# n7koirala/image_matching

Measured on AMD Instinct MI355X. Metric: encrypted DB vectors matched/sec (HyDia indexScenario, CKKS N=2^15), higher is better.
Workload: dtype u64

## Files before the change

### image_matching_amd/csrc/context.cpp

```cpp
#include <algorithm>
#include <cmath>
#include <cstdio>
#include <cstdlib>
#include <cstring>

#include <sys/stat.h>

#include "hydia_core.h"

namespace hydia {

u64 mulmod_u64(u64 a, u64 b, u64 q) { return (u64)(((u128)a * b) % q); }
u64 powmod_u64(u64 a, u64 e, u64 q) {
    u64 r = 1 % q;
    a %= q;
    for (; e; e >>= 1) {
        if (e & 1) r = mulmod_u64(r, a, q);
        a = mulmod_u64(a, a, q);
    }
    return r;
}
u64 invmod_u64(u64 a, u64 q) { return powmod_u64(a % q, q - 2, q); }

static bool miller_rabin(u64 n) {
// ... 336 lines not shown
        tabs.p2_wg_sync = getenv("HYDIA_P2_WG_SYNC") ? 1 : 0;
        tabs.no_tw_lds = getenv("HYDIA_NO_TW_LDS") ? 1 : 0;
    }
    modup_per_digit = getenv("HYDIA_MODUP_PER_DIGIT") != nullptr;
    loop_a_separate_ip = getenv("HYDIA_LOOPA_SEPARATE_IP") != nullptr;
    loop_a_int_ip = getenv("HYDIA_LOOPA_INT_IP") != nullptr;
    loop_a_limb_fastest = getenv("HYDIA_LOOPA_LIMB_FASTEST") != nullptr;
    relin_separate_intt = getenv("HYDIA_RELIN_SEPARATE_INTT") != nullptr;
    tabs.pm_mask = 0;
    if (!getenv("HYDIA_NTT_INT") && !getenv("HYDIA_NTT_NO_PM"))
        for (int m = 0; m < nT; m++)
            if (!((tabs.fp_mask >> m) & 1u) && mod[m].q < (1ull << 60) && (1ull << 60) - mod[m].q < (1ull << 24)) tabs.pm_mask |= 1u << m;
    if (const char *e = getenv("HYDIA_TENSOR_BPP")) tensor_bpp = std::max(1, atoi(e));
    if (const char *e = getenv("HYDIA_TENSOR_NW")) tensor_nw = atoi(e);
    merge_rescale = getenv("HYDIA_NO_MERGE_RESCALE") == nullptr;
    fuse_ip = getenv("HYDIA_NO_FUSE_IP") == nullptr;
    fork_products = getenv("HYDIA_NO_FORK") == nullptr;
    fuse_loop_a = getenv("HYDIA_NO_FUSE_LOOPA") == nullptr;
    colfuse = getenv("HYDIA_NO_COLFUSE") == nullptr;
    if (const char *e = getenv("HYDIA_MATVEC")) {
        if (e[0] == 'h') matvec_mode = 1;
        else if (e[0] == 'b') matvec_mode = bsgs_babies();
        else if (e[0] >= '1' && e[0] <= '9') matvec_mode = babies_for(1, atoi(e));
        else matvec_mode = 0;
    }
    rot_packed = getenv("HYDIA_KEYS_UNPACKED") == nullptr;
    db_packed = getenv("HYDIA_DB_UNPACKED") == nullptr;
    db_seq_ok = getenv("HYDIA_DB_CT_MAJOR") == nullptr;
    for (int j = 1; j < nQ; j++)
        if (q[j] >> 48) db_packed = false;
// ... 594 lines not shown
```

### image_matching_amd/csrc/evaluator.cpp

```cpp
#include <algorithm>
#include <cmath>
#include <cstring>

#include "hydia_core.h"

#include <exception>

namespace hydia {

static u64 shoup_h(u64 w, u64 q) { return (u64)(((u128)w << 64) / q); }

void op_bytes(const char *op, size_t N, double transforms, double other_bytes) {
    hk::ledger_add(op, transforms * 2.0 * (double)N * 8.0 + other_bytes);
}

void Context::ntt_fwd(u64 *base, size_t outer, int X, const LimbSel &s) {
    if (X <= 0 || s.n <= 0) return;
    hk::ntt_forward(stream, tabs, prm.logN, base, base, outer, outer, X, s);
}
void Context::ntt_inv(const u64 *src, u64 *dst, size_t so, size_t dso, int X, const LimbSel &s, const ScaleSel &sc) {
    if (X <= 0 || s.n <= 0) return;
    hk::ntt_inverse(stream, tabs, prm.logN, src, dst, so, dso, X, s, sc);
}

// ... 576 lines not shown
    relin_rescale_into(c, dbl, sub, addc, sub_is_add, out.d);
    c = std::move(out);
}
void Context::relin_rescale_into(const Ct &c, bool dbl, const Ct *sub, const double *addc, bool sub_is_add, u64 *out_d, const ProdSrc *ps,
                                 const ScaleSel *kap) {
    const int nl = c.nl, l = nl - 1;
    const int nE = nl + nP, nd = (nl + alpha - 1) / alpha, X = c.X, XP = X * 2;
    op_bytes("op:relin_rescale", N, (double)X * (nd * nE + 2 * nP + 4 * nl), (double)nd * 2 * nE * N * 8);
    u64 *dig = pool.get((size_t)X * nd * nE * N * sizeof(u64));
    u64 *d2buf = ps ? pool.get((size_t)X * nl * N * sizeof(u64)) : nullptr;
    const u64 *c2 = ps ? d2buf : c.d + 2 * c.poly_elems();
    const size_t c2_xs = ps ? (size_t)nl * N : c.ct_elems();
    const bool fip = fuse_ip;
    modup_digits(c2, c2_xs, X, nl, dig, false, fip, ps, d2buf);
    const LimbSel esel = sel_ext(nl);
    u64 *acc = pool.get((size_t)XP * nE * N * sizeof(u64));
    const size_t yu_outer = (size_t)(1 + nP) * N;
    u64 *yu = pool.get((size_t)XP * yu_outer * sizeof(u64));
    const bool tail_in_ip = !relin_separate_intt;
    const bool fused_tail = fip && tail_in_ip && prm.logN == 15;
    const LimbSel qsel_full = sel_q(nl);
    std::vector<u64> pinv(Pinv_mod_q.begin(), Pinv_mod_q.begin() + nl);
    const ScaleSel pinv_sel = scale_of(qsel_full, pinv, false);
    const DropLimb drop{l, dbl ? 1 : 0, pinv_sel.s[l], pinv_sel.s_sh[l], c.d, ps ? 0 : c.ct_elems(), ps ? 0 : c.poly_elems(), ps};
    bool drop_done = false;
    timer_begin("ks_inner_product");
    if (fip)
        drop_done = hk::ntt15_p2_inner_product(stream, tabs, d_mod, dig, (size_t)nd * nE * N, nd, X, nl, nP, nT, alpha, relin_key.d_cell, relin_key.d,
                                               c2, c2_xs, acc, fused_tail ? yu : nullptr, yu_outer, 1, fused_tail ? &drop : nullptr);
    else
        hk::inner_product(stream, d_mod, N, dig, (size_t)nd * nE * N, nd, relin_key.d_cell, 1, nT, acc, X, esel, c2, c2_xs, alpha, nl);
    timer_end("ks_inner_product");
    pool.put(dig);
    if (d2buf) pool.put(d2buf);
    if (ps && !(drop_done && fused_tail)) throw std::runtime_error("hydia: fused product outside the merged pipeline (prod_fusable out of step)");
    if (!fused_tail)
        hk::moddown_last_limb(stream, d_mod, N, acc, nE, c.d, c.ct_elems(), c.poly_elems(), acc + (size_t)l * N, (size_t)nE * N, XP, l,
                              pinv_sel.s[l], pinv_sel.s_sh[l], dbl ? 1 : 0);
    LimbSel tail{};
    tail.n = 1 + nP;
    tail.mod[0] = l;
    std::vector<u64> tail_scale(1 + nP, 1);
    for (int k = 0; k < nP; k++) {
        tail.mod[1 + k] = nQ + k;
        tail_scale[1 + k] = Phat_inv[k];
    }
    const bool cfu = cf_ok() && (q[l] >> 50) == 0;
    const bool cf_pre = cfu && cf_small_moddown(XP);
    if (fused_tail) {
        if (!drop_done)
            hk::ntt15_inverse_p2_last_limb(stream, tabs, acc + (size_t)l * N, yu, (size_t)nE * N, yu_outer, XP, l, pinv_sel.s[l], pinv_sel.s_sh[l],
                                           c.d, c.ct_elems(), c.poly_elems(), dbl ? 1 : 0);
        if (!cfu || cf_pre) hk::ntt15_inverse_p1(stream, tabs, yu, yu_outer, XP, tail, scale_of(tail, tail_scale, true));
    } else if (cfu && !cf_pre) {
        hk::ntt15_inverse_p2(stream, tabs, acc + (size_t)l * N, yu, (size_t)nE * N, yu_outer, XP, tail);
    } else {
        ntt_inv(acc + (size_t)l * N, yu, (size_t)nE * N, yu_outer, XP, tail, scale_of(tail, tail_scale, true));
    }
    const u64 *u = yu, *y = yu + N;
    ConvTab tab{};
    tab.ns = nP;
    tab.nt = nl;
// ... 6 lines not shown
    if (cfu) {
        const CfPlan &cp = cf_plan_moddown_rescale(nl, dbl);
        hk::ntt15_colfuse(stream, tabs, yu, yu_outer, w, (size_t)l * N, XP, cp.dev, cp.host.data(), 1, cf_pre);
    } else {
        hk::moddown_rescale_conv(stream, d_mod, N, y, yu_outer, u, yu_outer, w, XP, l, nP, tab);
    }
    const LimbSel qsel = sel_q(l);
    const double out_scale = c.scale / (double)q[l];
    std::vector<u64> qi(ql_inv[l].begin(), ql_inv[l].begin() + l);
    NttLoad ld{};
    NttStore stp{};
    stp.mode = 3;
    stp.out = out_d;
    stp.nl = l;
    stp.in = acc;
    stp.in_ls = nE;
    stp.mul = pinv_sel;
    stp.mul2 = scale_of(qsel, qi, false);
    stp.addend = c.d;
    stp.add_x = ps ? 0 : c.ct_elems();
    stp.add_p = ps ? 0 : c.poly_elems();
    stp.add_polys = 2;
    if (ps) {
        stp.has_prod = 1;
        stp.prod = *ps;
        if (ps->c) stp.kap = *kap;
    }
    stp.dbl = dbl ? 1 : 0;
    stp.sub = sub ? sub->d : nullptr;
    stp.sub_ls = sub ? sub->lstride : 0;
    stp.sub_add = sub_is_add ? 1 : 0;
    stp.has_addc = addc ? 1 : 0;
    stp.npoly = 2;
    if (addc)
        for (int j = 0; j < l; j++) stp.addc[j] = double_to_mod(*addc * out_scale, q[j]);
    if (cfu) hk::ntt15_forward_p2_fused(stream, tabs, w, (size_t)l * N, XP, qsel, stp);
    else hk::ntt15_forward_fused(stream, tabs, w, w, (size_t)l * N, (size_t)l * N, XP, qsel, ld, stp);
    pool.put(w);
    pool.put(yu);
    pool.put(acc);
}
Ct Context::clone(const Ct &a) {
    Ct o(this, a.X, a.npoly, a.nl, a.scale);
    hk::copy_limbs(stream, N, a.d, o.d, a.poly_elems(), o.poly_elems(), a.X * a.npoly, a.nl);
    return o;
}
void Context::drop_to(Ct &a, int nl) {
    if (nl < a.nl) a.nl = nl;
}
static void check_same(const Ct &a, const Ct &b, const char *what) {
    if (a.X != b.X || a.npoly != b.npoly || a.nl != b.nl)
// ... 952 lines not shown
```

### image_matching_amd/csrc/hydia_core.h

```cpp
#pragma once
#include <hip/hip_runtime.h>

#include <cstdint>
#include <cstdio>
#include <exception>
#include <map>
#include <mutex>
#include <memory>
#include <stdexcept>
#include <string>
#include <vector>

#include "kernels.h"

namespace hydia {
struct DeviceError : std::runtime_error {
    using std::runtime_error::runtime_error;
};
struct StateError : std::runtime_error {
    using std::runtime_error::runtime_error;
};
}

#define HIP_CHECK(expr)                                                                                   \
// ... 220 lines not shown
    void rescale(Ct &c, const Ct *sub = nullptr, const double *addc = nullptr);
    void relin_rescale(Ct &c, bool dbl = false, const Ct *sub = nullptr, const double *addc = nullptr, bool sub_is_add = false);
    bool ks_fused_ok() const { return prm.logN == 15 && fuse_ip && !relin_separate_intt && cf_ok() && ks_fuse; }
    bool rescale_cf = true;
    bool ks_fuse = true;
    void ks_fused(const u64 *c1, size_t c1_xs, int X, int nl, const u64 *key, const u64 *const *d_key_cell, const u64 *const *d_keys,
                  const u64 *addend, size_t add_x, size_t add_p, int add_polys, const unsigned *d_ginv, int same_g, bool dbl, u64 *out);
    void relin_rescale_into(const Ct &c, bool dbl, const Ct *sub, const double *addc, bool sub_is_add, u64 *out_d, const ProdSrc *ps = nullptr,
                            const ScaleSel *kap = nullptr);
    bool prod_fuse = true;
    bool prod_fusable(int nl) const;
    Ct mult_relin_rescale(const Ct &a, const Ct &b, bool dbl = false, const Ct *sub = nullptr, const double *addc = nullptr, bool sub_is_add = false,
                          const Ct *csub = nullptr);
    bool prod_fuse_csub = true;
    bool merge_rescale = true;
    Ct clone(const Ct &a);
    void drop_to(Ct &a, int nl);
    int tensor_bpp = 2;
    int tensor_nw = 4;
    bool modup_per_digit = false, loop_a_separate_ip = false, loop_a_int_ip = false, relin_separate_intt = false, loop_a_limb_fastest = false;
    void add_inplace(Ct &a, const Ct &b);
    void sub_inplace(Ct &a, const Ct &b);
    void add_const(Ct &a, double c);
    Ct mul_const(const Ct &a, double c, double const_scale);
    Ct lincomb(const std::vector<const Ct *> &terms, const std::vector<double> &coef, double c0, double S);
    Ct lincomb_multi(const std::vector<const Ct *> &terms, const std::vector<std::vector<double>> &coef, const std::vector<double> &c0,
                     const std::vector<double> &S);
    std::vector<std::vector<u64>> lcm_stage;
    Ct mult_norelin(const Ct &a, const Ct &b);
    Ct similarity_accumulate(const Ct &qc);
// ... 187 lines not shown
```

### image_matching_amd/csrc/ntt15.hip

```cpp
#include "kernels.h"
#include "ntt_arith.h"

#include <algorithm>
#include <cstdlib>
#include <type_traits>

namespace {

template <int LD>
DEV u64 p1_load(const NttLoad &ld, const ModC *__restrict__ mod, const ModC &M, const u64 *s, int x, int slot, size_t idx) {
    if (LD == 0) return s[idx];
    const u64 ql = mod[ld.l].q, v = ld.y[(size_t)x * ld.y_outer + idx];
    return v > (ql >> 1) ? negmod(reduce64(ql - v, M), M.q) : reduce64(v, M);
}

template <class A, int LD>
DEV typename A::T p1_load_as(const A &ar, const NttLoad &ld, const ModC *__restrict__ mod, const ModC &M, const u64 *s, int x, int slot,
                             size_t idx, std::integral_constant<int, LD>) {
    return ar.from_canon(p1_load<LD>(ld, mod, M, s, x, slot, idx));
}
DEV double p1_load_as(const FpA &ar, const NttLoad &ld, const ModC *__restrict__ mod, const ModC &M, const u64 *, int x, int, size_t idx,
                      std::integral_constant<int, 2>) {
    const u64 ql = mod[ld.l].q, v = ld.y[(size_t)x * ld.y_outer + idx];
    if (ql >> 50) {
// ... 322 lines not shown
    DEV u64 fin_lazy(const IntP &ar, const ModC &, int) const { return ar.fold128(s); }
};
template <>
struct IpAcc<FpA> {
    typedef double V;
    double s = 0;
    DEV static V prep(const FpA &ar, double c) {
        ar.recentre(c);
        return c;
    }
    DEV static V canon(u64 v) { return FpA::u2d(v); }
    DEV void mac(const FpA &ar, V v, u64 key) { s += ar.mulmod2(v, FpA::u2d(key)); }
    DEV u64 fin(const FpA &ar, const ModC &, int) const { return ar.fin_fwd(s); }
    DEV u64 fin_lazy(const FpA &ar, const ModC &M, int terms) const { return fin(ar, M, terms); }
};
template <int ST, class A>
DEV P2Pre p2_prefetch(const NttStore &st, const A &ar, int xp, int j, unsigned idx, const ModC &M) {
    constexpr size_t N = 32768;
    P2Pre r;
    r.has_ex = false;
    r.ex0 = r.ex1 = make_ulonglong2(0, 0);
    if (ST == 5) {
        loop_a_inner_product<false>(st.la, ar, M, xp >> 1, xp & 1, j, idx, r.in0, r.in1);
    } else {
        const u64 *pi = st.in + ((size_t)xp * st.in_ls + j) * N + idx;
        r.in0 = *reinterpret_cast<const ulonglong2 *>(pi);
        r.in1 = *reinterpret_cast<const ulonglong2 *>(pi + 2);
    }
    r.sb0 = r.sb1 = make_ulonglong2(0, 0);
    r.has_sb = false;
    if (ST == 1 || ST == 3 || ST == 5 || ST == 9 || ST == 10 || ST == 11) {
        const int x = xp >> 1, p = xp & 1;
        if (st.addend && p < st.add_polys && ST != 9 && ST != 10 && ST != 11) {
            const u64 *pa = st.addend + (size_t)x * st.add_x + (size_t)p * st.add_p + (size_t)j * N + idx;
            r.ex0 = *reinterpret_cast<const ulonglong2 *>(pa);
            r.ex1 = *reinterpret_cast<const ulonglong2 *>(pa + 2);
            r.has_ex = true;
        }
// ... 303 lines not shown
            ar.gs(v[p][0], v[p][2], W8a);
            ar.gs(v[p][1], v[p][3], W8a);
            ar.gs(v[p][4], v[p][6], W8b);
            ar.gs(v[p][5], v[p][7], W8b);
#pragma unroll
            for (int k = 0; k < 4; k++) ar.gs(v[p][k], v[p][k + 4], W7);
#pragma unroll
            for (int k = 0; k < 8; k++) {
                ar.recentre_wide(v[p][k]);
                d[p][blk * 256 + 32 * k + w] = A::to_bits(v[p][k]);
            }
        }
    }
}

template <class A, bool INV, int NP, int ST, bool SWZ = false, bool WGS = P2_WGS_DEFAULT>
DEV void p2_body(const A ar, const ulonglong2 *__restrict__ tw, const u64 *const *s, u64 *const *d, u64 (*lds)[P2Lds<SWZ>::SIZE], int t,
                 int B0, const NttStore &stp, const ModC &M, int xp0, int slot, const ulonglong2 *__restrict__ itw = nullptr,
                 u64 *const *dinv = nullptr, const P2Tab tab = P2Tab{nullptr, nullptr}) {
    typedef typename A::T T;
    typedef typename A::TW TW;
    typedef P2Lds<SWZ> LI;
    const int blk = t >> 5, w = t & 31;
    const int bg = (B0 >> 8) + blk;
    const int a = w >> 2, b = w & 3;
    const double *wt = nullptr;
    if (std::is_same<A, FpA>::value && !WGS && tab.g && tab.l) {
        double *wl = tab.l + (t >> 6) * 128;
        p2_stage_twiddles(tab.g, wl, (B0 >> 8) + 2 * (t >> 6), t & 63);
        wt = wl;
    }
    T v[NP][8];
    if (!INV) {
#pragma unroll
        for (int p = 0; p < NP; p++)
#pragma unroll
            for (int k = 0; k < 8; k++) v[p][k] = ar.from_raw(s[p][blk * 256 + 32 * k + w]);
        {
            if (wt) p2_sync<false>();
            TW W7, W8a, W8b, W9[4];
            p2_tw_A(ar, tw, wt, bg, blk & 1, W7, W8a, W8b, W9);
#pragma unroll
            for (int p = 0; p < NP; p++) {
#pragma unroll
// ... 28 lines not shown
                ar.ct(v[p][5], v[p][7], W11b);
#pragma unroll
                for (int k = 0; k < 8; k += 2) ar.ct(v[p][k], v[p][k + 1], W12[k >> 1]);
#pragma unroll
                for (int k = 0; k < 8; k++) lds[p][LI::at(blk, a, 4 * k + b)] = A::to_bits(v[p][k]);
            }
        }
        constexpr bool SPLIT = ST == 5 || ST == 3 || ST == 9 || ST == 10 || ST == 11;
        const Epi3Fp epi = Epi3Fp::make<ST, A>(stp, ar, M, slot);
        P2Pre pre[2][NP];
        P2Prod po;
        if (ST != 0 && ST != 4 && ST != 6) {
#pragma unroll
            for (int hh = 0; hh < (SPLIT ? 1 : 2); hh++)
#pragma unroll
                for (int p = 0; p < NP; p++) pre[hh][p] = p2_prefetch<ST>(stp, ar, xp0 + p, slot, (unsigned)(B0 + p2_elem<WGS>(t, hh)), M);
            if (ST == 9 || ST == 10 || ST == 11) po.load(stp.prod, xp0 >> 1, slot, (unsigned)(B0 + p2_elem<WGS>(t, 0)));
        }
        const u64 *const ip_key = (ST == 4 || ST == 6) ? (stp.ip.keys ? stp.ip.keys[xp0] : stp.ip.key) : nullptr;
        const int ip_t = slot, ip_m = ip_t < stp.ip.nl ? ip_t : stp.ip.nT - stp.ip.nE + ip_t;
        const int ip_own = (stp.ip.own && ip_t < stp.ip.nl) ? ip_t / stp.ip.alpha : (1 << 30);
        constexpr bool KB = (ST == 4 || ST == 6) && std::is_same<A, FpA>::value && !WGS;
        ulonglong2 kq[KB ? NP : 1][4];
        TW Wq[3];
        auto ip_request = [&](int hh) {
            const int e = p2_elem<WGS>(t, hh), gi = (B0 + e) >> 2;
            Wq[0] = A::tw(tw[8192 + gi]);
            Wq[1] = A::tw(tw[16384 + 2 * gi]);
            Wq[2] = A::tw(tw[16384 + 2 * gi + 1]);
#pragma unroll
            for (int p = 0; p < (KB ? NP : 1); p++) {
// ... 5 lines not shown
                kq[p][2] = *reinterpret_cast<const ulonglong2 *>(ka);
                kq[p][3] = *reinterpret_cast<const ulonglong2 *>(ka + 2);
            }
        };
        if (KB) ip_request(0);
        p2_sync<WGS>();
#pragma unroll
        for (int hh = 0; hh < 2; hh++) {
            const int e = p2_elem<WGS>(t, hh), u = e & 255, la = LI::at(e >> 8, u >> 5, u & 31);
            const int gi = (B0 + e) >> 2;
            if (KB && hh == 1) ip_request(1);
            const TW W13 = KB ? Wq[0] : A::tw(tw[8192 + gi]), W14a = KB ? Wq[1] : A::tw(tw[16384 + 2 * gi]), W14b = KB ? Wq[2] : A::tw(tw[16384 + 2 * gi + 1]);
            IpAcc<A> ipb[4], ipa[4];
            if (SPLIT && hh == 1) {
#pragma unroll
                for (int p = 0; p < NP; p++) pre[0][p] = p2_prefetch<ST>(stp, ar, xp0 + p, slot, (unsigned)(B0 + p2_elem<WGS>(t, 1)), M);
                if (ST == 9 || ST == 10 || ST == 11) po.load(stp.prod, xp0 >> 1, slot, (unsigned)(B0 + p2_elem<WGS>(t, 1)));
            }
#pragma unroll
            for (int p = 0; p < NP; p++) {
                T c0 = A::from_bits(lds[p][la]), c1 = A::from_bits(lds[p][la + 1]), c2 = A::from_bits(lds[p][la + 2]),
                  c3 = A::from_bits(lds[p][la + 3]);
                ar.mid(c0); ar.mid(c1); ar.mid(c2); ar.mid(c3);
                ar.ct(c0, c2, W13);
                ar.ct(c1, c3, W13);
                ar.ct(c0, c1, W14a);
                ar.ct(c2, c3, W14b);
                if (ST == 4 || ST == 6) {
                    const typename IpAcc<A>::V vv[4] = {IpAcc<A>::prep(ar, c0), IpAcc<A>::prep(ar, c1), IpAcc<A>::prep(ar, c2), IpAcc<A>::prep(ar, c3)};
                    const int dgt = p >= ip_own ? p + 1 : p;
                    const u64 *kb = ip_key + (((size_t)dgt * 2) * stp.ip.nT + ip_m) * 32768 + (B0 + e);
// ... 70 lines not shown
                                f4[k] = addmod(mulmod_shoup(f4[k], stp.ip.drop_mul, stp.ip.drop_mul_sh, qq), dv[k], qq);
                                if (stp.ip.drop_dbl) f4[k] = addmod(f4[k], f4[k], qq);
                            }
                        }
                        T c0 = ar.from_canon(f4[0]), c1 = ar.from_canon(f4[1]), c2 = ar.from_canon(f4[2]), c3 = ar.from_canon(f4[3]);
                        ar.gs(c0, c1, I14a);
                        ar.gs(c2, c3, I14b);
                        ar.gs(c0, c2, I13);
                        ar.gs(c1, c3, I13);
                        ar.recentre_wide(c0); ar.recentre_wide(c1); ar.recentre_wide(c2); ar.recentre_wide(c3);
                        lds[pp][la] = A::to_bits(c0); lds[pp][la + 1] = A::to_bits(c1);
                        lds[pp][la + 2] = A::to_bits(c2); lds[pp][la + 3] = A::to_bits(c3);
                    }
                    continue;
                }
                u64 *ob = stp.ip.acc + (((size_t)xp0 * 2) * stp.ip.nE + ip_t) * 32768 + ci;
                u64 *oa = ob + (size_t)stp.ip.nE * 32768;
                *reinterpret_cast<ulonglong2 *>(ob) = make_ulonglong2(ipb[0].fin(ar, M, NP + 1), ipb[1].fin(ar, M, NP + 1));
                *reinterpret_cast<ulonglong2 *>(ob + 2) = make_ulonglong2(ipb[2].fin(ar, M, NP + 1), ipb[3].fin(ar, M, NP + 1));
                *reinterpret_cast<ulonglong2 *>(oa) = make_ulonglong2(ipa[0].fin(ar, M, NP + 1), ipa[1].fin(ar, M, NP + 1));
                *reinterpret_cast<ulonglong2 *>(oa + 2) = make_ulonglong2(ipa[2].fin(ar, M, NP + 1), ipa[3].fin(ar, M, NP + 1));
            }
        }
        if (ST == 6) {
            p2_sync<WGS>();
            p2_inverse_BA<A, 2, SWZ, WGS>(ar, itw, lds, dinv, t, B0);
        }
    } else {
#pragma unroll
        for (int hh = 0; hh < 2; hh++) {
            const int e = p2_elem<WGS>(t, hh), u = e & 255, la = LI::at(e >> 8, u >> 5, u & 31);
            const int gi = (B0 + e) >> 2;
// ... 70 lines not shown
    const P2Tab tab{(fp && twg && !T.no_tw_lds) ? twg + (size_t)m * N : nullptr, &twl[0][0]};                                              \
    if (fp) p2_body<FpA, INV, NP, ST_, SWZ, WGS_>(FpA(M), tw, s, d, lds, threadIdx.x, B0, stp, M, xp * NP, slot, nullptr, nullptr, tab);   \
    else if ((T.pm_mask >> m) & 1u) p2_body<IntP, INV, NP, ST_, SWZ, WGS_>(IntP(M), tw, s, d, lds, threadIdx.x, B0, stp, M, xp * NP, slot); \
    else p2_body<IntA, INV, NP, ST_, SWZ, WGS_>(IntA(M), tw, s, d, lds, threadIdx.x, B0, stp, M, xp * NP, slot);
template <bool INV, int NP, int ST>
__global__ __launch_bounds__(256, (!INV && ST == 5) ? 3 : (!INV && ST == 10) ? 4 : 1) void k_ntt15_p2(NttTables T, const u64 *__restrict__ src, u64 *__restrict__ dst, size_t so,
                                                  size_t dso, LimbSel sel, int slot0, int nsl, NttStore stp) {
    P2_KERNEL_BODY(ST, P2_WGS_DEFAULT)
}
template <bool INV, int NP>
__global__ __launch_bounds__(256) void k_ntt15_p2_wgsync(NttTables T, const u64 *__restrict__ src, u64 *__restrict__ dst, size_t so, size_t dso, LimbSel sel,
                                                          int slot0, int nsl, NttStore stp) {
    P2_KERNEL_BODY(0, true)
}

template <int NP, bool OWN, bool TAIL, bool SWZ = false>
DEV void p2_ip_workgroup(const NttTables &T, const u64 *__restrict__ dig, size_t dxs, int t, int x, const NttStore &stp, int bx,
                         u64 (*lds)[P2Lds<SWZ>::SIZE], double *twl) {
    constexpr int N = 32768;
    const int m = t < stp.ip.nl ? t : stp.ip.nT - stp.ip.nE + t;
    const ModC M = T.mod[m];
    const bool fp = (T.fp_mask >> m) & 1u;
    const ulonglong2 *__restrict__ tw = (fp ? T.twf : T.twp) + (size_t)m * N;
    const int B0 = bx * 2048;
    const int own_d = OWN ? t / stp.ip.alpha : (1 << 30);
    const u64 *s[NP];
    u64 *d[NP];
#pragma unroll
    for (int p = 0; p < NP; p++) {
        const int dgt = p >= own_d ? p + 1 : p;
        s[p] = dig + (size_t)x * dxs + ((size_t)dgt * stp.ip.nE + t) * N + B0;
        d[p] = nullptr;
    }
    if (TAIL) {
        const ulonglong2 *__restrict__ itw = (fp ? T.itwf : T.itwp) + (size_t)m * N;
        u64 *dinv[2];
#pragma unroll
        for (int pp = 0; pp < 2; pp++)
            dinv[pp] = stp.ip.inv_out + (size_t)(2 * x + pp) * stp.ip.inv_outer + (size_t)(stp.ip.inv_row0 + t - stp.ip.nl) * N + B0;
        if (fp) p2_body<FpA, false, NP, 6, SWZ>(FpA(M), tw, s, d, lds, threadIdx.x, B0, stp, M, x, t, itw, dinv, P2Tab{(T.twd && !T.no_tw_lds) ? T.twd + (size_t)m * N : nullptr, twl});
        else if ((T.pm_mask >> m) & 1u) p2_body<IntP, false, NP, 6, SWZ>(IntP(M), tw, s, d, lds, threadIdx.x, B0, stp, M, x, t, itw, dinv);
        else p2_body<IntA, false, NP, 6, SWZ>(IntA(M), tw, s, d, lds, threadIdx.x, B0, stp, M, x, t, itw, dinv);
        return;
    }
    if (fp) p2_body<FpA, false, NP, 4, SWZ>(FpA(M), tw, s, d, lds, threadIdx.x, B0, stp, M, x, t, nullptr, nullptr, P2Tab{(T.twd && !T.no_tw_lds) ? T.twd + (size_t)m * N : nullptr, twl});
    else if ((T.pm_mask >> m) & 1u) p2_body<IntP, false, NP, 4, SWZ>(IntP(M), tw, s, d, lds, threadIdx.x, B0, stp, M, x, t);
    else p2_body<IntA, false, NP, 4, SWZ>(IntA(M), tw, s, d, lds, threadIdx.x, B0, stp, M, x, t);
}
template <int NP, bool OWN, bool TAIL = false>
__global__ __launch_bounds__(256) void k_ntt15_p2_ip(NttTables T, const u64 *__restrict__ dig, size_t dxs, int X, int t0, NttStore stp) {
    __shared__ u64 lds[(TAIL && NP < 2) ? 2 : NP][8 * 288];
    __shared__ double twl[4][128];
    const int slot = blockIdx.y / X, x = blockIdx.y - slot * X;
    p2_ip_workgroup<NP, OWN, TAIL>(T, dig, dxs, t0 + slot, x, stp, blockIdx.x, lds, &twl[0][0]);
}
template <int ND>
__global__ __launch_bounds__(256, ND == 2 ? 4 : 1) void k_ntt15_p2_ip_all(NttTables T, const u64 *__restrict__ dig, size_t dxs, int X, int xb, NttStore stp) {
    constexpr bool SWZ = ND >= 3;
    __shared__ u64 lds[ND][P2Lds<SWZ>::SIZE];
    __shared__ double twl[4][128];
    const int nl = stp.ip.nl, nS = stp.ip.nE, nP = nS - nl;
    const int per = nS * xb, grp = blockIdx.y / per, r = blockIdx.y - grp * per;
    const int si = r / xb, x = grp * xb + (r - si * xb);
    const int pc = si * nP / nS, pc1 = (si + 1) * nP / nS;
    if (pc1 > pc) p2_ip_workgroup<ND, false, true, SWZ>(T, dig, dxs, nl + pc, x, stp, blockIdx.x, lds, &twl[0][0]);
    else if (si - pc == stp.ip.drop_l) p2_ip_workgroup<ND - 1, true, true, SWZ>(T, dig, dxs, si - pc, x, stp, blockIdx.x, lds, &twl[0][0]);
    else p2_ip_workgroup<ND - 1, true, false, SWZ>(T, dig, dxs, si - pc, x, stp, blockIdx.x, lds, &twl[0][0]);
}


constexpr int OP_LDS_ELEMS = 512 * 33;

DEV int op_pin(int x) {
    asm volatile("" : "+v"(x));
    return x;
}
DEV FpA::TW op_tw(const FpA &, const ulonglong2 b) { return FpA::tw(b); }
DEV FpA::TW op_tw(const FpA &ar, const double wv) { return ar.tw8(wv); }
template <bool INV, class TWP>
DEV void op_stage_set(const FpA &ar, double (&v)[32], const TWP *__restrict__ tw, int base_shift, int hi, int nst, int first_bit) {
#pragma unroll
    for (int ss = 0; ss < nst; ss++) {
// ... 209 lines not shown
#pragma unroll
                    for (int k = 0; k < 32; k++) ar.recentre(w[k]);
                }
            }
            const u64 sc = scale.s[slot], scs = scale.s_sh[slot];
#pragma unroll
            for (int k = 0; k < 32; k++) d[(size_t)k * 1024 + t] = ar.fin_inv(w[k], sc, scs);
        }
    }
}

}

namespace hk {

bool ntt15_p2_inner_product(hipStream_t st, const NttTables &T, const ModC *mod, const u64 *dig, size_t dxs, int nd, int X, int nl,
                            int nP, int nT, int alpha, const u64 *const *keys, const u64 *key, const u64 *c2, size_t c2_xs, u64 *acc,
                            u64 *inv_out, size_t inv_outer, int inv_row0, const DropLimb *drop, bool per_x_keys) {
    const int nE = nl + nP;
    NttStore stp{};
    stp.mode = 4;
    stp.ip.key = key;
    stp.ip.keys = per_x_keys ? keys : nullptr;
    stp.ip.nT = nT;
    stp.ip.nE = nE;
    stp.ip.nl = nl;
    stp.ip.alpha = alpha;
    stp.ip.own = 1;
    stp.ip.c2 = c2;
    stp.ip.c2_xs = c2_xs;
    stp.ip.acc = acc;
    stp.ip.inv_out = inv_out;
    stp.ip.inv_outer = inv_outer;
    stp.ip.inv_row0 = inv_row0;
    stp.ip.drop_l = -1;
    const double bytes_q = nd >= 2 ? ((nd - 1) + 1 + 2.0) * nl * X * 262144.0 : 0.0, bytes_p = (nd + 2.0) * nP * X * 262144.0;
    const bool merged = inv_out && nd >= 2 && nd <= 4 && !T.two_ip_launches;
    char name[64];
    if (merged) {
        if (drop && !T.no_drop_in_ip && inv_row0 >= 1 && drop->l == nl - 1) {
            stp.ip.drop_l = drop->l;
            stp.ip.drop_dbl = drop->dbl;
            stp.ip.drop_mul = drop->mul;
            stp.ip.drop_mul_sh = drop->mul_sh;
            stp.ip.drop_add = drop->add;
            stp.ip.drop_add_x = drop->add_x;
            stp.ip.drop_add_p = drop->add_p;
            stp.ip.drop_has_prod = drop->prod ? 1 : 0;
            if (drop->prod) stp.ip.drop_prod = *drop->prod;
        }
        snprintf(name, sizeof name, "k_ntt15_p2_ip_all<%d>", nd);
        ledger_add(name, bytes_q + bytes_p);
        int xb = T.ip_group;
        if (xb < 1 || xb > X || X % xb) xb = X;
        if (nd == 2) hipLaunchKernelGGL((k_ntt15_p2_ip_all<2>), dim3(16, (nl + nP) * X), dim3(256), 0, st, T, dig, dxs, X, xb, stp);
        else if (nd == 3) hipLaunchKernelGGL((k_ntt15_p2_ip_all<3>), dim3(16, (nl + nP) * X), dim3(256), 0, st, T, dig, dxs, X, xb, stp);
        else hipLaunchKernelGGL((k_ntt15_p2_ip_all<4>), dim3(16, (nl + nP) * X), dim3(256), 0, st, T, dig, dxs, X, xb, stp);
        return stp.ip.drop_l >= 0;
    }
    if (nd >= 2) {
        snprintf(name, sizeof name, "k_ntt15_p2_ip<%d, true, false>", nd - 1 > 3 ? 3 : nd - 1);
        ledger_add(name, bytes_q);
    }
    snprintf(name, sizeof name, inv_out ? "k_ntt15_p2_ip<%d, false, true>" : "k_ntt15_p2_ip<%d, false, false>", nd > 4 ? 4 : nd);
    ledger_add(name, bytes_p);
// ... 252 lines not shown
```

Before: 19.99 million.

## Fuse Q-limb key-switch inner product into the rescale forward NTT epilogue

Splits the relinearisation inner product so that only the P limbs, the dropped last limb and limb 0 run in a tail kernel. The remaining Q-limb inner products are computed in registers inside a new kernel that immediately runs the rescale forward NTT and epilogue on them. This avoids writing and re-reading the full nE-limb accumulator, which shrinks to one limb per polynomial. In exchange the new kernel has higher register pressure and lower occupancy, and it applies only under a narrow set of conditions (X>=16, 2-3 digits, a particular fp_mask pattern).

```diff
diff --git a/image_matching_amd/csrc/context.cpp b/image_matching_amd/csrc/context.cpp
--- a/image_matching_amd/csrc/context.cpp
+++ b/image_matching_amd/csrc/context.cpp
@@ -374,6 +374,8 @@
     if (const char *e = getenv("HYDIA_TENSOR_BPP")) tensor_bpp = std::max(1, atoi(e));
     if (const char *e = getenv("HYDIA_TENSOR_NW")) tensor_nw = atoi(e);
     merge_rescale = getenv("HYDIA_NO_MERGE_RESCALE") == nullptr;
+    ipq_fuse = getenv("HYDIA_NO_IPQ_FUSE") == nullptr;
+    if (const char *e = getenv("HYDIA_IPQ_MIN")) ipq_min = std::max(1, atoi(e));
     fuse_ip = getenv("HYDIA_NO_FUSE_IP") == nullptr;
     fork_products = getenv("HYDIA_NO_FORK") == nullptr;
     fuse_loop_a = getenv("HYDIA_NO_FUSE_LOOPA") == nullptr;
diff --git a/image_matching_amd/csrc/evaluator.cpp b/image_matching_amd/csrc/evaluator.cpp
--- a/image_matching_amd/csrc/evaluator.cpp
+++ b/image_matching_amd/csrc/evaluator.cpp
@@ -3,6 +3,7 @@
 #include <cstring>
 
 #include "hydia_core.h"
+#include "ntt15_ipq.h"
 
 #include <exception>
 
@@ -614,25 +615,34 @@
     const bool fip = fuse_ip;
     modup_digits(c2, c2_xs, X, nl, dig, false, fip, ps, d2buf);
     const LimbSel esel = sel_ext(nl);
-    u64 *acc = pool.get((size_t)XP * nE * N * sizeof(u64));
+    const bool tail_in_ip = !relin_separate_intt;
+    const bool fused_tail = fip && tail_in_ip && prm.logN == 15;
+    const bool cfu = cf_ok() && (q[l] >> 50) == 0;
+    const bool ipq = ipq_fuse && X >= ipq_min && fused_tail && cfu && nd >= 2 && nd <= 3 && !(ps && ps->c) && !tabs.two_ip_launches &&
+                     !tabs.no_drop_in_ip && (tabs.fp_mask & ((1u << l) - 1u)) == ((1u << l) - 2u);
+    u64 *acc = pool.get((size_t)XP * (ipq ? 1 : nE) * N * sizeof(u64));
     const size_t yu_outer = (size_t)(1 + nP) * N;
     u64 *yu = pool.get((size_t)XP * yu_outer * sizeof(u64));
-    const bool tail_in_ip = !relin_separate_intt;
-    const bool fused_tail = fip && tail_in_ip && prm.logN == 15;
     const LimbSel qsel_full = sel_q(nl);
     std::vector<u64> pinv(Pinv_mod_q.begin(), Pinv_mod_q.begin() + nl);
     const ScaleSel pinv_sel = scale_of(qsel_full, pinv, false);
     const DropLimb drop{l, dbl ? 1 : 0, pinv_sel.s[l], pinv_sel.s_sh[l], c.d, ps ? 0 : c.ct_elems(), ps ? 0 : c.poly_elems(), ps};
+    const IpArgs ipa = hk::ntt15_ip_args(nl, nP, nT, alpha, relin_key.d_cell, relin_key.d, c2, c2_xs, acc, yu, yu_outer, 1, false);
     bool drop_done = false;
     timer_begin("ks_inner_product");
-    if (fip)
+    if (ipq) {
+        hk::ntt15_p2_ip_tail(stream, tabs, dig, (size_t)nd * nE * N, nd, X, ipa, drop);
+        drop_done = true;
+    } else if (fip)
         drop_done = hk::ntt15_p2_inner_product(stream, tabs, d_mod, dig, (size_t)nd * nE * N, nd, X, nl, nP, nT, alpha, relin_key.d_cell, relin_key.d,
                                                c2, c2_xs, acc, fused_tail ? yu : nullptr, yu_outer, 1, fused_tail ? &drop : nullptr);
     else
         hk::inner_product(stream, d_mod, N, dig, (size_t)nd * nE * N, nd, relin_key.d_cell, 1, nT, acc, X, esel, c2, c2_xs, alpha, nl);
     timer_end("ks_inner_product");
-    pool.put(dig);
-    if (d2buf) pool.put(d2buf);
+    if (!ipq) {
+        pool.put(dig);
+        if (d2buf) pool.put(d2buf);
+    }
     if (ps && !(drop_done && fused_tail)) throw std::runtime_error("hydia: fused product outside the merged pipeline (prod_fusable out of step)");
     if (!fused_tail)
         hk::moddown_last_limb(stream, d_mod, N, acc, nE, c.d, c.ct_elems(), c.poly_elems(), acc + (size_t)l * N, (size_t)nE * N, XP, l,
@@ -645,7 +655,6 @@
         tail.mod[1 + k] = nQ + k;
         tail_scale[1 + k] = Phat_inv[k];
     }
-    const bool cfu = cf_ok() && (q[l] >> 50) == 0;
     const bool cf_pre = cfu && cf_small_moddown(XP);
     if (fused_tail) {
         if (!drop_done)
@@ -682,7 +691,7 @@
     stp.out = out_d;
     stp.nl = l;
     stp.in = acc;
-    stp.in_ls = nE;
+    stp.in_ls = ipq ? 1 : nE;
     stp.mul = pinv_sel;
     stp.mul2 = scale_of(qsel, qi, false);
     stp.addend = c.d;
@@ -702,7 +711,13 @@
     stp.npoly = 2;
     if (addc)
         for (int j = 0; j < l; j++) stp.addc[j] = double_to_mod(*addc * out_scale, q[j]);
-    if (cfu) hk::ntt15_forward_p2_fused(stream, tabs, w, (size_t)l * N, XP, qsel, stp);
+    if (ipq) {
+        timer_begin("ks_inner_product");
+        hk::ntt15_p2_ipq(stream, tabs, dig, (size_t)nd * nE * N, nd, X, ipa, w, (size_t)l * N, stp);
+        timer_end("ks_inner_product");
+        pool.put(dig);
+        if (d2buf) pool.put(d2buf);
+    } else if (cfu) hk::ntt15_forward_p2_fused(stream, tabs, w, (size_t)l * N, XP, qsel, stp);
     else hk::ntt15_forward_fused(stream, tabs, w, w, (size_t)l * N, (size_t)l * N, XP, qsel, ld, stp);
     pool.put(w);
     pool.put(yu);
diff --git a/image_matching_amd/csrc/hydia_core.h b/image_matching_amd/csrc/hydia_core.h
--- a/image_matching_amd/csrc/hydia_core.h
+++ b/image_matching_amd/csrc/hydia_core.h
@@ -258,6 +258,8 @@
                           const Ct *csub = nullptr);
     bool prod_fuse_csub = true;
     bool merge_rescale = true;
+    bool ipq_fuse = true;
+    int ipq_min = 16;
     Ct clone(const Ct &a);
     void drop_to(Ct &a, int nl);
     int tensor_bpp = 2;
diff --git a/image_matching_amd/csrc/ntt15.hip b/image_matching_amd/csrc/ntt15.hip
--- a/image_matching_amd/csrc/ntt15.hip
+++ b/image_matching_amd/csrc/ntt15.hip
@@ -1,5 +1,6 @@
 #include "kernels.h"
 #include "ntt_arith.h"
+#include "ntt15_ipq.h"
 
 #include <algorithm>
 #include <cstdlib>
@@ -360,14 +361,17 @@
     DEV u64 fin(const FpA &ar, const ModC &, int) const { return ar.fin_fwd(s); }
     DEV u64 fin_lazy(const FpA &ar, const ModC &M, int terms) const { return fin(ar, M, terms); }
 };
-template <int ST, class A>
-DEV P2Pre p2_prefetch(const NttStore &st, const A &ar, int xp, int j, unsigned idx, const ModC &M) {
+template <int ST, class A, bool REGIN = false>
+DEV P2Pre p2_prefetch(const NttStore &st, const A &ar, int xp, int j, unsigned idx, const ModC &M, const u64 *rin = nullptr) {
     constexpr size_t N = 32768;
     P2Pre r;
     r.has_ex = false;
     r.ex0 = r.ex1 = make_ulonglong2(0, 0);
     if (ST == 5) {
         loop_a_inner_product<false>(st.la, ar, M, xp >> 1, xp & 1, j, idx, r.in0, r.in1);
+    } else if (REGIN) {
+        r.in0 = make_ulonglong2(rin[0], rin[1]);
+        r.in1 = make_ulonglong2(rin[2], rin[3]);
     } else {
         const u64 *pi = st.in + ((size_t)xp * st.in_ls + j) * N + idx;
         r.in0 = *reinterpret_cast<const ulonglong2 *>(pi);
@@ -701,10 +705,10 @@
     }
 }
 
-template <class A, bool INV, int NP, int ST, bool SWZ = false, bool WGS = P2_WGS_DEFAULT>
+template <class A, bool INV, int NP, int ST, bool SWZ = false, bool WGS = P2_WGS_DEFAULT, int IPQ = 0>
 DEV void p2_body(const A ar, const ulonglong2 *__restrict__ tw, const u64 *const *s, u64 *const *d, u64 (*lds)[P2Lds<SWZ>::SIZE], int t,
                  int B0, const NttStore &stp, const ModC &M, int xp0, int slot, const ulonglong2 *__restrict__ itw = nullptr,
-                 u64 *const *dinv = nullptr, const P2Tab tab = P2Tab{nullptr, nullptr}) {
+                 u64 *const *dinv = nullptr, const P2Tab tab = P2Tab{nullptr, nullptr}, u64 (*keep)[2][4] = nullptr) {
     typedef typename A::T T;
     typedef typename A::TW TW;
     typedef P2Lds<SWZ> LI;
@@ -714,7 +718,7 @@
     const double *wt = nullptr;
     if (std::is_same<A, FpA>::value && !WGS && tab.g && tab.l) {
         double *wl = tab.l + (t >> 6) * 128;
-        p2_stage_twiddles(tab.g, wl, (B0 >> 8) + 2 * (t >> 6), t & 63);
+        if (IPQ != 2) p2_stage_twiddles(tab.g, wl, (B0 >> 8) + 2 * (t >> 6), t & 63);
         wt = wl;
     }
     T v[NP][8];
@@ -773,7 +777,8 @@
 #pragma unroll
             for (int hh = 0; hh < (SPLIT ? 1 : 2); hh++)
 #pragma unroll
-                for (int p = 0; p < NP; p++) pre[hh][p] = p2_prefetch<ST>(stp, ar, xp0 + p, slot, (unsigned)(B0 + p2_elem<WGS>(t, hh)), M);
+                for (int p = 0; p < NP; p++)
+                    pre[hh][p] = p2_prefetch<ST, A, IPQ == 2>(stp, ar, xp0 + p, slot, (unsigned)(B0 + p2_elem<WGS>(t, hh)), M, IPQ == 2 ? keep[hh][p] : nullptr);
             if (ST == 9 || ST == 10 || ST == 11) po.load(stp.prod, xp0 >> 1, slot, (unsigned)(B0 + p2_elem<WGS>(t, 0)));
         }
         const u64 *const ip_key = (ST == 4 || ST == 6) ? (stp.ip.keys ? stp.ip.keys[xp0] : stp.ip.key) : nullptr;
@@ -809,7 +814,8 @@
             IpAcc<A> ipb[4], ipa[4];
             if (SPLIT && hh == 1) {
 #pragma unroll
-                for (int p = 0; p < NP; p++) pre[0][p] = p2_prefetch<ST>(stp, ar, xp0 + p, slot, (unsigned)(B0 + p2_elem<WGS>(t, 1)), M);
+                for (int p = 0; p < NP; p++)
+                    pre[0][p] = p2_prefetch<ST, A, IPQ == 2>(stp, ar, xp0 + p, slot, (unsigned)(B0 + p2_elem<WGS>(t, 1)), M, IPQ == 2 ? keep[1][p] : nullptr);
                 if (ST == 9 || ST == 10 || ST == 11) po.load(stp.prod, xp0 >> 1, slot, (unsigned)(B0 + p2_elem<WGS>(t, 1)));
             }
 #pragma unroll
@@ -910,8 +916,16 @@
                     }
                     continue;
                 }
-                u64 *ob = stp.ip.acc + (((size_t)xp0 * 2) * stp.ip.nE + ip_t) * 32768 + ci;
-                u64 *oa = ob + (size_t)stp.ip.nE * 32768;
+                if (IPQ == 1) {
+#pragma unroll
+                    for (int k = 0; k < 4; k++) {
+                        keep[hh][0][k] = ipb[k].fin(ar, M, NP + 1);
+                        keep[hh][1][k] = ipa[k].fin(ar, M, NP + 1);
+                    }
+                    continue;
+                }
+                u64 *ob = stp.ip.acc + (IPQ == 3 ? (size_t)xp0 * 2 : ((size_t)xp0 * 2) * stp.ip.nE + ip_t) * 32768 + ci;
+                u64 *oa = ob + (size_t)(IPQ == 3 ? 1 : stp.ip.nE) * 32768;
                 *reinterpret_cast<ulonglong2 *>(ob) = make_ulonglong2(ipb[0].fin(ar, M, NP + 1), ipb[1].fin(ar, M, NP + 1));
                 *reinterpret_cast<ulonglong2 *>(ob + 2) = make_ulonglong2(ipb[2].fin(ar, M, NP + 1), ipb[3].fin(ar, M, NP + 1));
                 *reinterpret_cast<ulonglong2 *>(oa) = make_ulonglong2(ipa[0].fin(ar, M, NP + 1), ipa[1].fin(ar, M, NP + 1));
@@ -1012,7 +1026,7 @@
     P2_KERNEL_BODY(0, true)
 }
 
-template <int NP, bool OWN, bool TAIL, bool SWZ = false>
+template <int NP, bool OWN, bool TAIL, bool SWZ = false, int IPQ = 0>
 DEV void p2_ip_workgroup(const NttTables &T, const u64 *__restrict__ dig, size_t dxs, int t, int x, const NttStore &stp, int bx,
                          u64 (*lds)[P2Lds<SWZ>::SIZE], double *twl) {
     constexpr int N = 32768;
@@ -1041,9 +1055,9 @@
         else p2_body<IntA, false, NP, 6, SWZ>(IntA(M), tw, s, d, lds, threadIdx.x, B0, stp, M, x, t, itw, dinv);
         return;
     }
-    if (fp) p2_body<FpA, false, NP, 4, SWZ>(FpA(M), tw, s, d, lds, threadIdx.x, B0, stp, M, x, t, nullptr, nullptr, P2Tab{(T.twd && !T.no_tw_lds) ? T.twd + (size_t)m * N : nullptr, twl});
-    else if ((T.pm_mask >> m) & 1u) p2_body<IntP, false, NP, 4, SWZ>(IntP(M), tw, s, d, lds, threadIdx.x, B0, stp, M, x, t);
-    else p2_body<IntA, false, NP, 4, SWZ>(IntA(M), tw, s, d, lds, threadIdx.x, B0, stp, M, x, t);
+    if (fp) p2_body<FpA, false, NP, 4, SWZ, P2_WGS_DEFAULT, IPQ>(FpA(M), tw, s, d, lds, threadIdx.x, B0, stp, M, x, t, nullptr, nullptr, P2Tab{(T.twd && !T.no_tw_lds) ? T.twd + (size_t)m * N : nullptr, twl});
+    else if ((T.pm_mask >> m) & 1u) p2_body<IntP, false, NP, 4, SWZ, P2_WGS_DEFAULT, IPQ>(IntP(M), tw, s, d, lds, threadIdx.x, B0, stp, M, x, t);
+    else p2_body<IntA, false, NP, 4, SWZ, P2_WGS_DEFAULT, IPQ>(IntA(M), tw, s, d, lds, threadIdx.x, B0, stp, M, x, t);
 }
 template <int NP, bool OWN, bool TAIL = false>
 __global__ __launch_bounds__(256) void k_ntt15_p2_ip(NttTables T, const u64 *__restrict__ dig, size_t dxs, int X, int t0, NttStore stp) {
@@ -1064,6 +1078,55 @@
     if (pc1 > pc) p2_ip_workgroup<ND, false, true, SWZ>(T, dig, dxs, nl + pc, x, stp, blockIdx.x, lds, &twl[0][0]);
     else if (si - pc == stp.ip.drop_l) p2_ip_workgroup<ND - 1, true, true, SWZ>(T, dig, dxs, si - pc, x, stp, blockIdx.x, lds, &twl[0][0]);
     else p2_ip_workgroup<ND - 1, true, false, SWZ>(T, dig, dxs, si - pc, x, stp, blockIdx.x, lds, &twl[0][0]);
+}
+
+template <int ND>
+__global__ __launch_bounds__(256, ND == 2 ? 4 : 1) void k_ntt15_p2_ip_tail(NttTables T, const u64 *__restrict__ dig, size_t dxs, int X, int xb, NttStore stp) {
+    constexpr bool SWZ = ND >= 3;
+    __shared__ u64 lds[ND][P2Lds<SWZ>::SIZE];
+    __shared__ double twl[4][128];
+    const int nl = stp.ip.nl, nP = stp.ip.nE - nl;
+    const int per = (nP + 2) * xb, grp = blockIdx.y / per, r = blockIdx.y - grp * per;
+    const int si = r / xb, x = grp * xb + (r - si * xb);
+    if (si < nP) p2_ip_workgroup<ND, false, true, SWZ>(T, dig, dxs, nl + si, x, stp, blockIdx.x, lds, &twl[0][0]);
+    else if (si == nP) p2_ip_workgroup<ND - 1, true, false, SWZ, 3>(T, dig, dxs, 0, x, stp, blockIdx.x, lds, &twl[0][0]);
+    else p2_ip_workgroup<ND - 1, true, true, SWZ>(T, dig, dxs, stp.ip.drop_l, x, stp, blockIdx.x, lds, &twl[0][0]);
+}
+template <int ND, int ST>
+__global__ __launch_bounds__(256, 3) void k_ntt15_p2_ipq(NttTables T, const u64 *__restrict__ dig, size_t dxs, u64 *__restrict__ w, size_t wso, int X, NttStore stp) {
+    constexpr int N = 32768, NP = ND - 1;
+    static_assert(ND == 2 || ND == 3, "one or two foreign digits: two padded LDS images serve both transforms");
+    constexpr bool SWZ = false, WGS = P2_WGS_DEFAULT;
+    __shared__ u64 lds[2][P2Lds<SWZ>::SIZE];
+    __shared__ double twl[4][128];
+    const int j = blockIdx.y / X, x = blockIdx.y - j * X, m = j, t = threadIdx.x;
+    const ModC M = T.mod[m];
+    const bool fp = (T.fp_mask >> m) & 1u;
+    const ulonglong2 *__restrict__ tw = (fp ? T.twf : T.twp) + (size_t)m * N;
+    const int B0 = blockIdx.x * 2048;
+    const u64 *ws[2];
+    u64 *wd[2];
+#pragma unroll
+    for (int p = 0; p < 2; p++) ws[p] = wd[p] = w + (size_t)(2 * x + p) * wso + (size_t)j * N + B0;
+    if (!fp) {
+        if ((T.pm_mask >> m) & 1u) p2_body<IntP, false, 2, ST, SWZ, WGS>(IntP(M), tw, ws, wd, lds, t, B0, stp, M, 2 * x, j);
+        else p2_body<IntA, false, 2, ST, SWZ, WGS>(IntA(M), tw, ws, wd, lds, t, B0, stp, M, 2 * x, j);
+        return;
+    }
+    const int own_d = j / stp.ip.alpha;
+    const u64 *s[NP];
+    u64 *d[NP];
+#pragma unroll
+    for (int p = 0; p < NP; p++) {
+        const int dgt = p >= own_d ? p + 1 : p;
+        s[p] = dig + (size_t)x * dxs + ((size_t)dgt * stp.ip.nE + j) * N + B0;
+        d[p] = nullptr;
+    }
+    u64 keep[2][2][4];
+    const P2Tab tab{(T.twd && !T.no_tw_lds) ? T.twd + (size_t)m * N : nullptr, &twl[0][0]};
+    p2_body<FpA, false, NP, 4, SWZ, WGS, 1>(FpA(M), tw, s, d, lds, t, B0, stp, M, x, j, nullptr, nullptr, tab, keep);
+    p2_sync<WGS>();
+    p2_body<FpA, false, 2, ST, SWZ, WGS, 2>(FpA(M), tw, ws, wd, lds, t, B0, stp, M, 2 * x, j, nullptr, nullptr, tab, keep);
 }
 
 
@@ -1303,41 +1366,89 @@
 
 namespace hk {
 
+static void ip_set_drop(IpArgs &ip, const DropLimb &drop) {
+    ip.drop_l = drop.l;
+    ip.drop_dbl = drop.dbl;
+    ip.drop_mul = drop.mul;
+    ip.drop_mul_sh = drop.mul_sh;
+    ip.drop_add = drop.add;
+    ip.drop_add_x = drop.add_x;
+    ip.drop_add_p = drop.add_p;
+    ip.drop_has_prod = drop.prod ? 1 : 0;
+    if (drop.prod) ip.drop_prod = *drop.prod;
+}
+
+void ntt15_p2_ip_tail(hipStream_t st, const NttTables &T, const u64 *dig, size_t dxs, int nd, int X, const IpArgs &ip, const DropLimb &drop) {
+    NttStore stp{};
+    stp.mode = 4;
+    stp.ip = ip;
+    ip_set_drop(stp.ip, drop);
+    const int nP = ip.nE - ip.nl;
+    char name[64];
+    snprintf(name, sizeof name, "k_ntt15_p2_ip_tail<%d>", nd);
+    ledger_add(name, ((nd + 2.0) * nP + 2 * ((nd - 1) + 1 + 2.0)) * X * 262144.0);
+    int xb = T.ip_group;
+    if (xb < 1 || xb > X || X % xb) xb = X;
+    const dim3 grid(16, (nP + 2) * X);
+    if (nd == 2) hipLaunchKernelGGL((k_ntt15_p2_ip_tail<2>), grid, dim3(256), 0, st, T, dig, dxs, X, xb, stp);
+    else hipLaunchKernelGGL((k_ntt15_p2_ip_tail<3>), grid, dim3(256), 0, st, T, dig, dxs, X, xb, stp);
+}
+template <int ST>
+static void launch_p2_ipq(hipStream_t st, const NttTables &T, const u64 *dig, size_t dxs, int nd, int X, u64 *w, size_t wso, const NttStore &sv) {
+    const int rows = sv.ip.nl - 1;
+    char name[64];
+    snprintf(name, sizeof name, "k_ntt15_p2_ipq<%d, %d>", nd, ST);
+    const double epi = 2.0 * (2.0 + (ST == 3 ? 2.0 : ST == 9 ? 3.0 : 4.0));
+    if (nd < 2 || nd > 3) throw std::runtime_error("hydia: ntt15_p2_ipq takes two or three digits");
+    ledger_add(name, (epi + (rows - 1) * (epi - 2.0 + nd)) * X * 262144.0);
+    const dim3 grid(16, rows * X);
+    if (nd == 2) hipLaunchKernelGGL((k_ntt15_p2_ipq<2, ST>), grid, dim3(256), 0, st, T, dig, dxs, w, wso, X, sv);
+    else hipLaunchKernelGGL((k_ntt15_p2_ipq<3, ST>), grid, dim3(256), 0, st, T, dig, dxs, w, wso, X, sv);
+}
+void ntt15_p2_ipq(hipStream_t st, const NttTables &T, const u64 *dig, size_t dxs, int nd, int X, const IpArgs &ip, u64 *w, size_t wso, const NttStore &epi) {
+    NttStore sv = epi;
+    sv.ip = ip;
+    sv.ip.drop_l = -1;
+    sv.int_epilogue = T.int_epilogue;
+    if (epi.has_prod && epi.prod.c) throw std::runtime_error("hydia: ntt15_p2_ipq has no epilogue with a product subtrahend");
+    if (epi.has_prod && epi.sub) launch_p2_ipq<10>(st, T, dig, dxs, nd, X, w, wso, sv);
+    else if (epi.has_prod) launch_p2_ipq<9>(st, T, dig, dxs, nd, X, w, wso, sv);
+    else launch_p2_ipq<3>(st, T, dig, dxs, nd, X, w, wso, sv);
+}
+
+IpArgs ntt15_ip_args(int nl, int nP, int nT, int alpha, const u64 *const *keys, const u64 *key, const u64 *c2, size_t c2_xs, u64 *acc, u64 *inv_out,
+                     size_t inv_outer, int inv_row0, bool per_x_keys) {
+    IpArgs ip{};
+    ip.key = key;
+    ip.keys = per_x_keys ? keys : nullptr;
+    ip.nT = nT;
+    ip.nE = nl + nP;
+    ip.nl = nl;
+    ip.alpha = alpha;
+    ip.own = 1;
+    ip.c2 = c2;
+    ip.c2_xs = c2_xs;
+    ip.acc = acc;
+    ip.inv_out = inv_out;
+    ip.inv_outer = inv_outer;
+    ip.inv_row0 = inv_row0;
+    ip.drop_l = -1;
+    return ip;
+}
+
 bool ntt15_p2_inner_product(hipStream_t st, const NttTables &T, const ModC *mod, const u64 *dig, size_t dxs, int nd, int X, int nl,
                             int nP, int nT, int alpha, const u64 *const *keys, const u64 *key, const u64 *c2, size_t c2_xs, u64 *acc,
                             u64 *inv_out, size_t inv_outer, int inv_row0, const DropLimb *drop, bool per_x_keys) {
     const int nE = nl + nP;
     NttStore stp{};
     stp.mode = 4;
-    stp.ip.key = key;
-    stp.ip.keys = per_x_keys ? keys : nullptr;
-    stp.ip.nT = nT;
-    stp.ip.nE = nE;
-    stp.ip.nl = nl;
-    stp.ip.alpha = alpha;
-    stp.ip.own = 1;
-    stp.ip.c2 = c2;
-    stp.ip.c2_xs = c2_xs;
-    stp.ip.acc = acc;
-    stp.ip.inv_out = inv_out;
-    stp.ip.inv_outer = inv_outer;
-    stp.ip.inv_row0 = inv_row0;
-    stp.ip.drop_l = -1;
+    stp.ip = ntt15_ip_args(nl, nP, nT, alpha, keys, key, c2, c2_xs, acc, inv_out, inv_outer, inv_row0, per_x_keys);
     const double bytes_q = nd >= 2 ? ((nd - 1) + 1 + 2.0) * nl * X * 262144.0 : 0.0, bytes_p = (nd + 2.0) * nP * X * 262144.0;
     const bool merged = inv_out && nd >= 2 && nd <= 4 && !T.two_ip_launches;
     char name[64];
     if (merged) {
-        if (drop && !T.no_drop_in_ip && inv_row0 >= 1 && drop->l == nl - 1) {
-            stp.ip.drop_l = drop->l;
-            stp.ip.drop_dbl = drop->dbl;
-            stp.ip.drop_mul = drop->mul;
-            stp.ip.drop_mul_sh = drop->mul_sh;
-            stp.ip.drop_add = drop->add;
-            stp.ip.drop_add_x = drop->add_x;
-            stp.ip.drop_add_p = drop->add_p;
-            stp.ip.drop_has_prod = drop->prod ? 1 : 0;
-            if (drop->prod) stp.ip.drop_prod = *drop->prod;
-        }
+        if (drop && !T.no_drop_in_ip && inv_row0 >= 1 && drop->l == nl - 1)
+            ip_set_drop(stp.ip, *drop);
         snprintf(name, sizeof name, "k_ntt15_p2_ip_all<%d>", nd);
         ledger_add(name, bytes_q + bytes_p);
         int xb = T.ip_group;
diff --git a/image_matching_amd/csrc/ntt15_ipq.h b/image_matching_amd/csrc/ntt15_ipq.h
--- /dev/null
+++ b/image_matching_amd/csrc/ntt15_ipq.h
@@ -0,0 +1,12 @@
+#pragma once
+#include "kernels.h"
+
+namespace hk {
+
+IpArgs ntt15_ip_args(int nl, int nP, int nT, int alpha, const u64 *const *keys, const u64 *key, const u64 *c2, size_t c2_xs, u64 *acc, u64 *inv_out,
+                     size_t inv_outer, int inv_row0, bool per_x_keys);
+void ntt15_p2_ip_tail(hipStream_t st, const NttTables &T, const u64 *dig, size_t dig_x_stride, int nd, int X, const IpArgs &ip, const DropLimb &drop);
+void ntt15_p2_ipq(hipStream_t st, const NttTables &T, const u64 *dig, size_t dig_x_stride, int nd, int X, const IpArgs &ip, u64 *w, size_t w_outer,
+                  const NttStore &epi);
+
+}
```

After: 20.28 million (median of 6 runs). +1.4%, better.
